# TUMFTM/global_racetrajectory_optimization

Hardware: NVIDIA H100
Metric: min-curv QPs/sec (N=1000 closed track, batched) (higher is better)
Workload: dtype f64

## Files before the change

global_racetrajectory_optimization_b200/batch.py:

```python
from __future__ import annotations

import ctypes
import functools
import math
from typing import Optional, Union

import torch

from . import _lib

_GRID_Y_MAX = 65535
N_MIN = 80
STATUS_TEXT = {
    0: "ok",
    1: "Problem not solvable, track might be too small to run with current safety distance!",
    2: "interior-point iteration cap reached",
    3: "numerical breakdown (non-positive pivot)",
    4: "curvature rows still violated after the curvature-row phase (constraints inconsistent)",
    -1: "unsupported track size",
}

F_SCALE = 2.0
VP_DECEL_SLICE_UPPER = 1

_WS = {}

SLAB_VECTORS = ("H DIAG DFW DBW LFW INVD TII RHOP RHOM PX PY NX NY MX MY XP YP SX SY KREF LB UB F "
                "T0 T1 T2 T3 T4 T5 ALPHA LU LL RD RHS DX DD DLU DLL SU SL ISU ISL HBSRC "
                "S3 S4 L3 L4 KL WK EDX T3K T4K VV IH").split()
HB_PITCH = 34
ZB_PITCH = 108


def mincurv_slab_layout(n_max: int) -> dict:
    np_ = ((n_max + 31) // 32) * 32 + 64
    nb_max = max(1, (n_max - 32 + 31) // 32)
    o = len(SLAB_VECTORS) * np_
    o_zb = o
    o += n_max * ZB_PITCH
    o_hb = o
    o += np_ * HB_PITCH
    o_tiles = o
    o += np_ * 67
    return dict(np=np_, nb_max=nb_max, o_zb=o_zb, o_hb=o_hb, o_tiles=o_tiles, stride=(o + 15) & ~15)


def _require_cuda() -> None:
    if not torch.cuda.is_available():
        raise _lib.MinCurvLibError("global_racetrajectory_optimization_b200 needs a CUDA device (H100, sm_90a); "
                                   "there is no CPU fallback")


def _ptr(t: Optional[torch.Tensor]):
    return ctypes.c_void_p(t.data_ptr()) if t is not None else None


def _stream():
    return ctypes.c_void_p(torch.cuda.current_stream().cuda_stream)


def _device_guard(fn):
    @functools.wraps(fn)
    def wrapper(*args, **kwargs):
        dev = next((a.device for a in list(args) + list(kwargs.values()) if isinstance(a, torch.Tensor) and a.is_cuda), None)
        if dev is None:
            return fn(*args, **kwargs)
# ... 697 lines not shown
```

global_racetrajectory_optimization_b200/csrc/mincurv_ipm.cu:

```cuda
#include <cstdio>
#include <cstdlib>
#include "mincurv_ops.cuh"

namespace mc {

constexpr unsigned FULL = 0xffffffffu;
constexpr int IP_THREADS = 64;
constexpr int SUB = 8;
constexpr int VBP = 12;
constexpr int FROW = 34;
constexpr int HB_SLOTS = 2;
constexpr int HO_SLOTS = 2;
constexpr int LROW = 33;
#ifndef MC_LT_SLOTS
#define MC_LT_SLOTS 3
#endif
constexpr int LT_SLOTS = MC_LT_SLOTS;
constexpr int GT_SLOTS = 6 - LT_SLOTS;
constexpr int RING_UNITS = LT_SLOTS + GT_SLOTS;
constexpr int QDEPTH = 16;
constexpr int LT_UNIT_DOUBLES = SUB * LROW;
constexpr int GT_UNIT_DOUBLES = SUB * FROW;
constexpr unsigned HB_UNIT_BYTES = SUB * HB_PITCH * sizeof(double);

__device__ __forceinline__ void dmma(double (&c)[2], double a, double b) {
    asm volatile("mma.sync.aligned.m8n8k4.row.col.f64.f64.f64.f64 {%0,%1}, {%2}, {%3}, {%0,%1};\n"
                 : "+d"(c[0]), "+d"(c[1]) : "d"(a), "d"(b));
}

__device__ __forceinline__ uint32_t smem_u32(const void *p) { return (uint32_t)__cvta_generic_to_shared(p); }
__device__ __forceinline__ void mbar_init(uint64_t *bar, unsigned count) {
    asm volatile("mbarrier.init.shared::cta.b64 [%0], %1;" ::"r"(smem_u32(bar)), "r"(count) : "memory");
}
__device__ __forceinline__ void mbar_expect_tx(uint64_t *bar, unsigned bytes) {
    asm volatile("mbarrier.arrive.expect_tx.shared::cta.b64 _, [%0], %1;" ::"r"(smem_u32(bar)), "r"(bytes) : "memory");
}
__device__ __forceinline__ void mbar_arrive(uint64_t *bar) {
    asm volatile("mbarrier.arrive.shared::cta.b64 _, [%0];" ::"r"(smem_u32(bar)) : "memory");
}
#ifndef MC_WAIT_MODE
#define MC_WAIT_MODE 1
#endif
#ifndef MC_RELAXED_BACKOFF_NS
#define MC_RELAXED_BACKOFF_NS 250
#endif
// ... 92 lines not shown
            double lt[LT_SLOTS][LT_UNIT_DOUBLES];
            double gt[GT_SLOTS][GT_UNIT_DOUBLES];
            double q[QDEPTH * SUB];
        } sw;
        double win[hband_win_doubles(IP_THREADS)];
    } u;
    union {
        double Ss[32 * 33];
        double sfrag[20 * 32];
    } s;
    double wS[32], gs[32], part[2][32];
    double red[32];
    uint64_t hb_full[HB_SLOTS], ho_full[HO_SLOTS], ho_empty[HO_SLOTS], ring_full[RING_UNITS];
    unsigned ring_phase[2];
    int prog[4];
    int flag;
    int next;
};

struct Factor {
    const double *HB;
    const double *DD;
    double *LT, *GT;
    int n, NA;
};

__device__ __forceinline__ Factor make_factor(double *slab, const Layout &L, int n, const double *HB) {
    Factor F;
    F.HB = HB;
    F.DD = vec(slab, L, V_DD);
    F.LT = slab + L.o_tiles;
    F.GT = F.LT + (size_t)L.np * LROW;
    F.n = n;
    F.NA = n - 32;
    return F;
}

__device__ __forceinline__ int lt_slot(int c, int m) { return LROW * c + ((m + 3 * c - 1) & 31); }
__device__ __forceinline__ double lt_entry(const double *unit, int c, int m) {
    return (c < m && m <= c + 32) ? unit[lt_slot(c, m)] : 0.0;
}

__device__ __forceinline__ int blk(int I, int J) { return (I * (I + 1)) / 2 + J; }

__device__ __noinline__ bool factor_chain(IpShared &sh, const double *__restrict__ HBp, const double *__restrict__ DD, double *__restrict__ LTp, double *__restrict__ GTp, const int NA, const double *__restrict__ g, unsigned tick) {
    const int lane = threadIdx.x & 31;
    const int gq = lane >> 2, q = lane & 3;
    const int nunits = (NA + SUB - 1) / SUB;
    const uint64_t pol = l2_evict_normal_policy();
    double W[10][2];
#pragma unroll
    for (int b = 0; b < 10; ++b) { W[b][0] = 0.0; W[b][1] = 0.0; }
    double gv = (lane < NA) ? g[lane] : 0.0;
    double gcur = (32 + lane < NA) ? g[32 + lane] : 0.0;
    double gnext = (64 + lane < NA) ? g[64 + lane] : 0.0;
    double ddcur = (lane < NA) ? DD[lane] : 0.0;
    double ddnext = (32 + lane < NA) ? DD[32 + lane] : 0.0;
    bool ok = true;
    if (lane == 0) {
        mbar_expect_tx(&sh.hb_full[tick % HB_SLOTS], HB_UNIT_BYTES);
        tma_load_1d(sh.u.f.hb[tick % HB_SLOTS], HBp, HB_UNIT_BYTES, &sh.hb_full[tick % HB_SLOTS], pol);
    }
    SEG_BEGIN();
    for (int t = 0; t < nunits; ++t) {
// ... 111 lines not shown
            }
        }
#pragma unroll
        for (int I = 0; I < 4; ++I)
#pragma unroll
            for (int J = 0; J <= I; ++J) {
                double c[2] = {0.0, 0.0};
                if (I < 3) { c[0] = W[blk(I + 1, J + 1)][0]; c[1] = W[blk(I + 1, J + 1)][1]; }
                dmma(c, af[I][0], bf[J][0]);
                dmma(c, af[I][1], bf[J][1]);
                W[blk(I, J)][0] = c[0]; W[blk(I, J)][1] = c[1];
            }
        {
            const double up = __shfl_sync(FULL, gv, (lane + 8) & 31), en = __shfl_sync(FULL, gv2, (lane - 24) & 31);
            gv = (lane < 24) ? up : en;
        }
        __syncwarp();
        SEG(12);
        if (lane == 0) mbar_arrive(&sh.ho_full[ls]);
    }
    return ok;
}

__device__ __noinline__ void factor_fill(IpShared &sh, const double *__restrict__ HBp, double *__restrict__ LTp, double *__restrict__ GTp, const int NA, const double *__restrict__ g, unsigned tick) {
    const int lane = threadIdx.x & 31;
    const int gq = lane >> 2, q = lane & 3;
    const int nunits = (NA + SUB - 1) / SUB;
    double G[4][4][2];
#pragma unroll
    for (int I = 0; I < 4; ++I)
#pragma unroll
        for (int J = 0; J < 4; ++J) { G[I][J][0] = 0.0; G[I][J][1] = 0.0; }
    double gsacc = 0.0;
    double *gb = sh.u.f.gb;
    for (int t = 0; t < nunits; ++t) {
        const unsigned ht = tick + t, ls = ht % HO_SLOTS;
        const int k0 = t * SUB;
#pragma unroll
        for (int I = 0; I < 4; ++I)
            *reinterpret_cast<double2 *>(&gb[(8 * I + gq) * VBP + 2 * q]) = make_double2(G[I][0][0], G[I][0][1]);
        __syncwarp();
        double gp[8];
#pragma unroll
        for (int j = 0; j < 8; j += 2) {
            const double2 uu = *reinterpret_cast<const double2 *>(&gb[lane * VBP + j]);
            gp[j] = uu.x; gp[j + 1] = uu.y;
        }
// ... 2 lines not shown
#pragma unroll
            for (int j = 0; j < 8; ++j) {
                const int k = k0 + j;
                double yv = 0.0;
                if (k < NA) {
                    if (k <= lane) yv = HBp[(size_t)(NA + lane) * HB_PITCH + (k + 32 - lane)];
                    else if (k >= NA + lane - 32) yv = HBp[(size_t)k * HB_PITCH + (NA + lane - k)];
                }
                gp[j] = yv - gp[j];
            }
        } else {
#pragma unroll
            for (int j = 0; j < 8; ++j) gp[j] = -gp[j];
        }
        __syncwarp();
        PROF_T0(tw2);
        mbar_wait_relaxed(&sh.ho_full[ls], (ht / HO_SLOTS) & 1u);
        PROF_ADD1(20, tw2);
        const Handoff &ho = sh.u.f.ho[ls];
#pragma unroll
        for (int m = 0; m < 7; ++m)
#pragma unroll
            for (int j = m + 1; j < 8; ++j) gp[j] = fma(-gp[m], ho.l11[j * 8 + m], gp[j]);
        double *gtp = GTp + (size_t)k0 * FROW;
#pragma unroll
        for (int j = 0; j < 8; ++j) {
            st_stream(gtp + j * FROW + lane, gp[j]);
            gsacc = fma(gp[j], ho.w[j] * ho.y[j], gsacc);
        }
        if (lane < 8) {
            const double w = ho.w[lane];
            *reinterpret_cast<double2 *>(gtp + lane * FROW + 32) = make_double2(w * ho.y[lane], w);
        }
#pragma unroll
        for (int j = 0; j < 8; j += 2) *reinterpret_cast<double2 *>(&gb[lane * VBP + j]) = make_double2(gp[j], gp[j + 1]);
        __syncwarp();
        PROF_T0(tw3);
        double af[4][2], bf[4][2], wq[2];
#pragma unroll
        for (int ks = 0; ks < 2; ++ks) {
            wq[ks] = ho.w[4 * ks + q];
#pragma unroll
            for (int I = 0; I < 4; ++I) {
                af[I][ks] = gb[(8 * I + gq) * VBP + 4 * ks + q];
                bf[I][ks] = ho.vb[(8 * I + gq) * VBP + 4 * ks + q];
            }
        }
#pragma unroll
        for (int I = 0; I < 4; ++I)
#pragma unroll
            for (int J = 0; J < 4; ++J) {
                double c[2] = {0.0, 0.0};
                if (J < 3) { c[0] = G[I][J + 1][0]; c[1] = G[I][J + 1][1]; }
                dmma(c, af[I][0], bf[J][0]);
                dmma(c, af[I][1], bf[J][1]);
// ... 17 lines not shown
            for (int J = 0; J <= I; ++J)
                *reinterpret_cast<double2 *>(&sh.s.sfrag[(blk(I, J) * 32 + lane) * 2]) = make_double2(c2[J][0], c2[J][1]);
        }
        __syncwarp();
        PROF_ADD1(21, tw3);
        if (lane == 0) mbar_arrive(&sh.ho_empty[ls]);
    }
    sh.gs[lane] = g[NA + lane] - gsacc;
}

__device__ __forceinline__ unsigned factor_units(int n) { return (unsigned)((n - 32 + SUB - 1) / SUB); }
__device__ __noinline__ bool factor(IpShared &sh, double *slab, const Layout &L, int n, const double *HB, const double *g, unsigned tick) {
    const Factor F = make_factor(slab, L, n, HB);
    const int NA = F.NA;
    const int warp = threadIdx.x >> 5, lane = threadIdx.x & 31;
    for (int e = threadIdx.x; e < 20 * 32; e += IP_THREADS) sh.s.sfrag[e] = 0.0;
    fence_proxy_async();
    __syncthreads();
    PROF_T0(tc0);
    if (warp == 0) {
        if (!factor_chain(sh, F.HB, F.DD, F.LT, F.GT, NA, g, tick)) sh.flag = 1;
        PROF_ADD(1, tc0);
    } else {
        factor_fill(sh, F.HB, F.LT, F.GT, NA, g, tick);
        PROF_ADD1(13, tc0);
    }
    PROF_T0(tc1);
    double sf[20];
    if (warp == 1) {
#pragma unroll
        for (int e = 0; e < 20; ++e) sf[e] = sh.s.sfrag[((e >> 1) * 32 + lane) * 2 + (e & 1)];
    }
    double sv[16];
#pragma unroll
    for (int i = 0; i < 16; ++i) {
        const int e = threadIdx.x + i * IP_THREADS;
        const int r = e >> 5, c = e & 31;
        const int lo = min(r, c), dist = abs(r - c);
        sv[i] = F.HB[(size_t)(NA + lo) * HB_PITCH + dist];
        if (r == c) sv[i] += F.DD[NA + r];
    }
    __syncthreads();
#pragma unroll
    for (int i = 0; i < 16; ++i) {
        const int e = threadIdx.x + i * IP_THREADS;
        sh.s.Ss[(e >> 5) * 33 + (e & 31)] = sv[i];
    }
// ... 58 lines not shown
        phase ^= 1u << sl;
        return buf + sl * UNIT_DOUBLES;
    }
    __device__ __forceinline__ void close() { sh.ring_phase[WHO] = phase; }
};
using LtRing = RingT<LT_SLOTS, 0, LT_UNIT_DOUBLES, 0>;
using GtRing = RingT<GT_SLOTS, LT_SLOTS, GT_UNIT_DOUBLES, 1>;

__device__ __forceinline__ void prog_publish(int *p, int v) { asm volatile("st.release.cta.shared.s32 [%0], %1;" ::"r"(smem_u32(p)), "r"(v) : "memory"); }
__device__ __forceinline__ int prog_read(const int *p) {
    int v;
    asm volatile("ld.acquire.cta.shared.s32 %0, [%1];" : "=r"(v) : "r"(smem_u32(p)) : "memory");
    return v;
}
template <bool BACKOFF = false>
__device__ __forceinline__ void prog_wait(IpShared &sh, const int *p, int need) {
    for (int spin = 0; spin < (1 << 18); ++spin) {
        if (prog_read(p) >= need) return;
        if (BACKOFF) __nanosleep(MC_RELAXED_BACKOFF_NS);
    }
    sh.flag = 1;
}

__device__ __noinline__ void sweep_forward(IpShared &sh, const double *__restrict__ HBp, double *__restrict__ LTp, double *__restrict__ GTp, const int NA, const double *__restrict__ g) {
    const int lane = threadIdx.x & 31;
    const int gq = lane >> 2, q = lane & 3;
    const int nunits = (NA + SUB - 1) / SUB;
    constexpr int AHEAD = LT_SLOTS - 1;
    LtRing R(sh, &sh.u.sw.lt[0][0]);
    if (lane == 0)
        for (int u = 0; u < AHEAD && u < nunits; ++u) R.issue(u, u, LTp);
    double acc[4];
#pragma unroll
    for (int I = 0; I < 4; ++I) acc[I] = (8 * I + gq < NA) ? g[8 * I + gq] : 0.0;
    double gcur = (32 + lane < NA) ? g[32 + lane] : 0.0;
    double gnext = (64 + lane < NA) ? g[64 + lane] : 0.0;
    int sl = 0, sn = AHEAD % LT_SLOTS;
    for (int u = 0; u < nunits; ++u, sl = (sl == LT_SLOTS - 1) ? 0 : sl + 1, sn = (sn == LT_SLOTS - 1) ? 0 : sn + 1) {
        const int k0 = u * SUB;
        if (u > 0 && (u & 3) == 0) {
            gcur = gnext;
            const int idx = k0 + 64 + lane;
            gnext = (idx < NA) ? g[idx] : 0.0;
        }
        if ((u & 7) == 0 && u >= 8) prog_wait(sh, &sh.prog[1], u - 8);
        const double *lt = R.wait(sl);
        const double ge = __shfl_sync(FULL, gcur, ((u & 3) << 3) + gq);
// ... 3 lines not shown
            a[I][0] = lt_entry(lt, q, 8 * I + gq);
            a[I][1] = lt_entry(lt, 4 + q, 8 * I + gq);
        }
        const double wl = lt[gq * LROW + 32];
        const double b0 = __shfl_sync(FULL, acc[0], 4 * q), b1 = __shfl_sync(FULL, acc[0], 16 + 4 * q);
        double y0[2] = {acc[0], acc[0]}, y1[2] = {0.0, 0.0};
        dmma(y0, a[0][0], b0);
        dmma(y1, a[0][1], b1);
        const double y = y0[0] + y1[0];
        const double n0 = -__shfl_sync(FULL, y, 4 * q), n1 = -__shfl_sync(FULL, y, 16 + 4 * q);
        double nw[4];
#pragma unroll
        for (int I = 0; I < 4; ++I) {
            const double c = (I < 3) ? acc[I + 1] : ge;
            double c0[2] = {c, c}, c1[2] = {0.0, 0.0};
            dmma(c0, a[I + 1][0], n0);
            dmma(c1, a[I + 1][1], n1);
            nw[I] = c0[0] + c1[0];
        }
        if (q == 0) {
            const bool in = (k0 + gq < NA);
            const double z = in ? y * wl : 0.0;
            sh.u.sw.q[(u & (QDEPTH - 1)) * SUB + gq] = z;
            if (in) GTp[(size_t)(k0 + gq) * FROW + 32] = z;
        }
#pragma unroll
        for (int I = 0; I < 4; ++I) acc[I] = nw[I];
        __syncwarp();
        if (lane == 0) {
            prog_publish(&sh.prog[0], u + 1);
            if (u + AHEAD < nunits) R.issue(u + AHEAD, sn, LTp);
        }
    }
    R.close();
    fence_proxy_async();
}

__device__ __noinline__ void sweep_sep_rhs(IpShared &sh, const double *__restrict__ HBp, double *__restrict__ LTp, double *__restrict__ GTp, const int NA, const double *__restrict__ g) {
    const int lane = threadIdx.x & 31;
    const int nunits = (NA + SUB - 1) / SUB;
    constexpr int AHEAD = GT_SLOTS - 1;
    GtRing R(sh, &sh.u.sw.gt[0][0]);
    if (lane == 0)
        for (int u = 0; u < AHEAD && u < nunits; ++u) R.issue(u, u, GTp);
    double s0 = 0.0, s1 = 0.0;
    const double gsl = g[NA + lane];
    int sl = 0, sn = AHEAD % GT_SLOTS;
    for (int u = 0; u < nunits; ++u, sl = (sl == GT_SLOTS - 1) ? 0 : sl + 1, sn = (sn == GT_SLOTS - 1) ? 0 : sn + 1) {
        const double *gt = R.wait(sl) + lane;
        prog_wait<true>(sh, &sh.prog[0], u + 1);
        const double *zq = &sh.u.sw.q[(u & (QDEPTH - 1)) * SUB];
#pragma unroll
        for (int s2 = 0; s2 < SUB; s2 += 2) {
            s0 = fma(gt[s2 * FROW], zq[s2], s0);
            s1 = fma(gt[(s2 + 1) * FROW], zq[s2 + 1], s1);
        }
        __syncwarp();
        if (lane == 0) {
            prog_publish(&sh.prog[1], u + 1);
            if (u + AHEAD < nunits) R.issue(u + AHEAD, sn, GTp);
        }
    }
    R.close();
    sh.gs[lane] = gsl - (s0 + s1);
}

__device__ __noinline__ void sweep_sep_solve(IpShared &sh, const double *__restrict__ HBp, double *__restrict__ LTp, double *__restrict__ GTp, const int NA, double *__restrict__ x) {
    const int lane = threadIdx.x & 31;
    const int nunits = (NA + SUB - 1) / SUB;
    constexpr int AHEAD = GT_SLOTS - 1;
    GtRing R(sh, &sh.u.sw.gt[0][0]);
    const int U0 = nunits - 1;
    if (lane == 0)
        for (int i = 0; i < AHEAD && i < nunits; ++i) R.issue(U0 - i, i, GTp);
    double a = sh.gs[lane];
#pragma unroll 4
    for (int k = 0; k < 32; ++k) {
        const double yk = __shfl_sync(FULL, a, k);
        const double l = (lane > k) ? sh.s.Ss[lane * 33 + k] : 0.0;
        a = fma(-l, yk, a);
    }
    a *= sh.wS[lane];
#pragma unroll 4
    for (int k = 31; k >= 0; --k) {
        const double xk = __shfl_sync(FULL, a, k);
        const double l = (lane < k) ? sh.s.Ss[k * 33 + lane] : 0.0;
        a = fma(-l, xk, a);
    }
    x[NA + lane] = a;
    const int kl = lane & 7, qr = lane >> 3;
    double xq[8];
#pragma unroll
    for (int i = 0; i < 8; ++i) xq[i] = __shfl_sync(FULL, a, 8 * qr + i);
    int sl = 0, sn = AHEAD % GT_SLOTS;
    for (int i = 0; i < nunits; ++i, sl = (sl == GT_SLOTS - 1) ? 0 : sl + 1, sn = (sn == GT_SLOTS - 1) ? 0 : sn + 1) {
        const int k = (U0 - i) * SUB + kl;
        if ((i & 7) == 0 && i >= 8) prog_wait<true>(sh, &sh.prog[2], i - 8);
        const double *gt = R.wait(sl) + kl * FROW;
        const double2 zw = *reinterpret_cast<const double2 *>(&gt[32]);
        double c0 = 0.0, c1 = 0.0;
#pragma unroll
        for (int e = 0; e < 8; e += 2) {
            const double2 gg = *reinterpret_cast<const double2 *>(&gt[8 * qr + e]);
            c0 = fma(gg.x, xq[e], c0);
            c1 = fma(gg.y, xq[e + 1], c1);
        }
        double c = c0 + c1;
        c += __shfl_xor_sync(FULL, c, 8);
        c += __shfl_xor_sync(FULL, c, 16);
        if (qr == 0) sh.u.sw.q[(i & (QDEPTH - 1)) * SUB + kl] = (k < NA) ? fma(-c, zw.y, zw.x) : 0.0;
        __syncwarp();
        if (lane == 0) {
            prog_publish(&sh.prog[3], i + 1);
            if (i + AHEAD < nunits) R.issue(U0 - i - AHEAD, sn, GTp);
        }
    }
    R.close();
}

__device__ __noinline__ void sweep_backward(IpShared &sh, const double *__restrict__ HBp, double *__restrict__ LTp, double *__restrict__ GTp, const int NA, double *__restrict__ x) {
    const int lane = threadIdx.x & 31;
    const int gq = lane >> 2, q = lane & 3;
    const int nunits = (NA + SUB - 1) / SUB;
    constexpr int AHEAD = LT_SLOTS - 1;
    LtRing R(sh, &sh.u.sw.lt[0][0]);
    const int U0 = nunits - 1;
    if (lane == 0)
        for (int i = 0; i < AHEAD && i < nunits; ++i) R.issue(U0 - i, i, LTp);
    double nbx[8];
#pragma unroll
    for (int i = 0; i < 8; ++i) nbx[i] = 0.0;
    int sl = 0, sn = AHEAD % LT_SLOTS;
    for (int i = 0; i < nunits; ++i, sl = (sl == LT_SLOTS - 1) ? 0 : sl + 1, sn = (sn == LT_SLOTS - 1) ? 0 : sn + 1) {
        const int k0 = (U0 - i) * SUB;
        const double *lt = R.wait(sl);
        double a[10];
#pragma unroll
        for (int c = 0; c < 10; ++c) a[c] = lt_entry(lt, gq, 4 * c + q);
        double c0[2] = {0.0, 0.0}, c1[2] = {0.0, 0.0};
#pragma unroll
        for (int e = 2; e < 8; e += 2) {
            dmma(c0, a[2 + e], nbx[e]);
            dmma(c1, a[3 + e], nbx[e + 1]);
        }
        dmma(c0, a[2], nbx[0]);
        dmma(c1, a[3], nbx[1]);
        prog_wait(sh, &sh.prog[3], i + 1);
        const double t1 = sh.u.sw.q[(i & (QDEPTH - 1)) * SUB + gq];
        const double uu = t1 + (c0[0] + c1[0]);
        const double u0 = __shfl_sync(FULL, uu, 4 * q), u1 = __shfl_sync(FULL, uu, 16 + 4 * q);
        double d0[2] = {uu, uu}, d1[2] = {0.0, 0.0};
        dmma(d0, a[0], u0);
        dmma(d1, a[1], u1);
        const double x1 = d0[0] + d1[0];
        if (q == 0 && k0 + gq < NA) x[k0 + gq] = x1;
#pragma unroll
        for (int e = 7; e >= 2; --e) nbx[e] = nbx[e - 2];
        nbx[0] = -__shfl_sync(FULL, x1, 4 * q);
        nbx[1] = -__shfl_sync(FULL, x1, 16 + 4 * q);
        __syncwarp();
        if (lane == 0) {
            prog_publish(&sh.prog[2], i + 1);
            if (i + AHEAD < nunits) R.issue(U0 - i - AHEAD, sn, LTp);
        }
    }
    R.close();
}

__device__ __noinline__ void solve(IpShared &sh, double *slab, const Layout &L, int n, const double *g, double *x, bool fused) {
    const Factor F = make_factor(slab, L, n, nullptr);
    const int warp = threadIdx.x >> 5;
    if (threadIdx.x < 4) sh.prog[threadIdx.x] = 0;
    fence_proxy_async();
    __syncthreads();
    if (!fused) {
        PROF_T0(t0);
        if (warp == 0) sweep_forward(sh, F.HB, F.LT, F.GT, F.NA, g);
        else sweep_sep_rhs(sh, F.HB, F.LT, F.GT, F.NA, g);
        __syncthreads();
        PROF_ADD1(2, t0);
    }
    PROF_T0(t3);
    if (warp == 1) sweep_sep_solve(sh, F.HB, F.LT, F.GT, F.NA, x);
    else sweep_backward(sh, F.HB, F.LT, F.GT, F.NA, x);
    __syncthreads();
    PROF_ADD1(8, t3);
}

__device__ void band_matvec(const double *__restrict__ HB, const double *__restrict__ v, double *__restrict__ out, int n) {
    for (int i = threadIdx.x; i < n; i += IP_THREADS) {
        const double *row = HB + (size_t)i * HB_PITCH;
        double s = row[0] * v[i];
        int j = i;
        for (int k = 1; k <= HBW; ++k) {
            j = (j + 1 == n) ? 0 : j + 1;
            s = fma(row[k], v[j], s);
        }
        j = i;
        for (int k = 1; k <= HBW; ++k) {
            j = (j == 0) ? n - 1 : j - 1;
            s = fma(HB[(size_t)j * HB_PITCH + k], v[j], s);
        }
        out[i] = s;
    }
}

__device__ __forceinline__ void ip_init_shared(IpShared &sh) {
    if (threadIdx.x == 0) {
        for (int i = 0; i < HB_SLOTS; ++i) mbar_init(&sh.hb_full[i], 1);
        for (int i = 0; i < HO_SLOTS; ++i) { mbar_init(&sh.ho_full[i], 1); mbar_init(&sh.ho_empty[i], 1); }
        for (int i = 0; i < RING_UNITS; ++i) mbar_init(&sh.ring_full[i], 1);
        sh.ring_phase[0] = 0; sh.ring_phase[1] = 0;
        asm volatile("fence.mbarrier_init.release.cluster;" ::: "memory");
    }
    __syncthreads();
}

__global__ void __launch_bounds__(IP_THREADS, 8)
mincurv_pdip_kernel(int B, int n_max, const int32_t *__restrict__ n_pts, double *__restrict__ ws, Layout L,
                    PdipParams prm, double *__restrict__ alpha_out, int32_t *__restrict__ status,
                    int32_t *__restrict__ iters_out, int *__restrict__ work_counter) {
    extern __shared__ __align__(16) unsigned char smem_raw[];
    IpShared &sh = *reinterpret_cast<IpShared *>(smem_raw);
#ifdef MC_DEBUG_SM_LIMIT
    {
        unsigned smid;
        asm volatile("mov.u32 %0, %%smid;" : "=r"(smid));
        if (smid >= MC_DEBUG_SM_LIMIT) return;
    }
#endif
    ip_init_shared(sh);
    unsigned tick = 0;

    for (;;) {
        __syncthreads();
        if (threadIdx.x == 0) sh.next = atomicAdd(work_counter, 1);
        __syncthreads();
        const int b = sh.next;
        if (b >= B) break;
        const int n = n_pts ? n_pts[b] : n_max;
        double *aout = alpha_out + (size_t)b * n_max;
        if (status[b] != 0) {
            for (int i = threadIdx.x; i < n_max; i += IP_THREADS) aout[i] = 0.0;
            if (iters_out && threadIdx.x == 0) iters_out[b] = 0;
            continue;
        }
        PROF_T0(tq0);
        double *slab = ws + (size_t)b * L.stride;
        const double *HB = ws + (size_t)*band_owner(slab, L) * L.stride + L.o_hb;
        const double *__restrict__ LB = vec(slab, L, V_LB), *__restrict__ UB = vec(slab, L, V_UB), *__restrict__ F = vec(slab, L, V_F);
        double *__restrict__ AL = vec(slab, L, V_ALPHA), *__restrict__ LU = vec(slab, L, V_LU), *__restrict__ LL = vec(slab, L, V_LL), *__restrict__ RD = vec(slab, L, V_RD);
        double *__restrict__ RHS = vec(slab, L, V_RHS), *__restrict__ DX = vec(slab, L, V_DX), *__restrict__ DD = vec(slab, L, V_DD);
        double *__restrict__ TU = vec(slab, L, V_DLU), *__restrict__ TL = vec(slab, L, V_DLL), *__restrict__ SU = vec(slab, L, V_SU), *__restrict__ SL = vec(slab, L, V_SL);
        double *__restrict__ ISU = vec(slab, L, V_ISU), *__restrict__ ISL = vec(slab, L, V_ISL);
        double *G0 = vec(slab, L, V_T0);
        if (threadIdx.x == 0) sh.flag = 0;

        for (int i = threadIdx.x; i < n; i += IP_THREADS) AL[i] = 0.5 * (LB[i] + UB[i]);
        __syncthreads();
        band_matvec(HB, AL, G0, n);
        __syncthreads();
        double gmax = 0.0, fmaxv = 0.0;
#pragma unroll 1
        for (int i = threadIdx.x; i < n; i += IP_THREADS) {
            const double gi = G0[i] + F[i];
            G0[i] = gi;
            gmax = fmax(gmax, fabs(gi));
            fmaxv = fmax(fmaxv, fabs(F[i]));
        }
        gmax = block_reduce<1>(gmax, sh.red);
        fmaxv = block_reduce<1>(fmaxv, sh.red);
        const double lam0 = prm.lam0_rel * gmax + 1e-300;
        double musum = 0.0;
#pragma unroll 1
        for (int i = threadIdx.x; i < n; i += IP_THREADS) {
            const double gi = G0[i];
            const double lu = fmax(-gi, 0.0) + lam0, ll = fmax(gi, 0.0) + lam0;
            const double rd = gi + lu - ll;
            LU[i] = lu; LL[i] = ll;
            RD[i] = rd;
            const double a = AL[i];
            const double su = UB[i] - a, sl = a - LB[i];
            const double isu = 1.0 / su, isl = 1.0 / sl;
            SU[i] = su; SL[i] = sl;
            ISU[i] = isu; ISL[i] = isl;
            DD[i] = lu * isu + ll * isl; RHS[i] = -rd + lu - ll;
            musum += su * lu + sl * ll;
        }
        musum = block_reduce<0>(musum, sh.red);
        const double mu0 = musum / (2.0 * n);
        const double rd_tol = prm.rd_rel * (fmaxv + gmax) + 1e-300;
        double mu = mu0;
        int it = 0;
        int result = 2;

        constexpr int VG = 4, VS = VG * IP_THREADS;
        for (it = 0; it < prm.max_iter; ++it) {
            PROF_T0(tf0);
            const bool fok = factor(sh, slab, L, n, HB, RHS, tick);
            tick += factor_units(n);
            if (!fok) { result = 3; break; }
            PROF_ADD(10, tf0);
            PROF_T0(ts0);
            solve(sh, slab, L, n, RHS, DX, true);
            PROF_ADD(6, ts0);
            PROF_T0(tv2);
            double rp = 0.0, rdl = 0.0, c00 = 0.0, c01 = 0.0, c10 = 0.0, c11 = 0.0;
#pragma unroll 1
            for (int i0 = threadIdx.x; i0 < n; i0 += VS) {
                double su[VG], sl[VG], lu[VG], ll[VG], dx[VG], isu[VG], isl[VG];
#pragma unroll
                for (int k = 0; k < VG; ++k) {
                    const int i = min(i0 + k * IP_THREADS, n - 1);
                    su[k] = SU[i]; sl[k] = SL[i]; lu[k] = LU[i]; ll[k] = LL[i]; dx[k] = DX[i]; isu[k] = ISU[i]; isl[k] = ISL[i];
                }
#pragma unroll
                for (int k = 0; k < VG; ++k) {
                    if (i0 + k * IP_THREADS < n) {
                        const double p = dx[k] * isu[k], m = dx[k] * isl[k];
                        rp = fmax(rp, fmax(p, -m));
                        rdl = fmax(rdl, fmax(1.0 - p, 1.0 + m));
                        const double dlu = lu[k] * (p - 1.0), dll = -ll[k] * (1.0 + m);
                        c00 += su[k] * lu[k] + sl[k] * ll[k];
                        c01 += su[k] * dlu + sl[k] * dll;
                        c10 += dx[k] * (ll[k] - lu[k]);
                        c11 += dx[k] * (dll - dlu);
                    }
                }
            }
            rp = block_reduce<1>(rp, sh.red);
            rdl = block_reduce<1>(rdl, sh.red);
            double ap = (rp > 1.0) ? 1.0 / rp : 1.0, ad = (rdl > 1.0) ? 1.0 / rdl : 1.0;
            c00 = block_reduce<0>(c00, sh.red); c01 = block_reduce<0>(c01, sh.red);
            c10 = block_reduce<0>(c10, sh.red); c11 = block_reduce<0>(c11, sh.red);
            const double mua = (c00 + ad * c01 + ap * c10 + ap * ad * c11) / (2.0 * n);
            double sigma = mua / mu;
            sigma = sigma * sigma * sigma;
            const double smu = sigma * mu;
            PROF_ADD(17, tv2);
            PROF_T0(tv3);
#pragma unroll 1
            for (int i0 = threadIdx.x; i0 < n; i0 += VS) {
                double su[VG], sl[VG], lu[VG], ll[VG], dx[VG], isu[VG], isl[VG], rd[VG];
#pragma unroll
                for (int k = 0; k < VG; ++k) {
                    const int i = min(i0 + k * IP_THREADS, n - 1);
                    su[k] = SU[i]; sl[k] = SL[i]; lu[k] = LU[i]; ll[k] = LL[i]; dx[k] = DX[i]; isu[k] = ISU[i]; isl[k] = ISL[i]; rd[k] = RD[i];
                }
#pragma unroll
                for (int k = 0; k < VG; ++k) {
                    const int i = i0 + k * IP_THREADS;
                    if (i < n) {
                        const double dlu = lu[k] * (dx[k] * isu[k] - 1.0), dll = -ll[k] * (1.0 + dx[k] * isl[k]);
                        const double tu = smu - su[k] * lu[k] + dx[k] * dlu;
                        const double tl = smu - sl[k] * ll[k] - dx[k] * dll;
                        TU[i] = tu; TL[i] = tl;
                        RHS[i] = -rd[k] - tu * isu[k] + tl * isl[k];
                    }
                }
            }
            __syncthreads();
            PROF_ADD(18, tv3);
            PROF_T0(ts1);
            solve(sh, slab, L, n, RHS, DX, false);
            PROF_ADD(7, ts1);
            PROF_T0(tv4);
            rp = 0.0; rdl = 0.0;
#pragma unroll 1
            for (int i0 = threadIdx.x; i0 < n; i0 += VS) {
                double lu[VG], ll[VG], dx[VG], isu[VG], isl[VG], tu[VG], tl[VG];
#pragma unroll
                for (int k = 0; k < VG; ++k) {
                    const int i = min(i0 + k * IP_THREADS, n - 1);
                    lu[k] = LU[i]; ll[k] = LL[i]; dx[k] = DX[i]; isu[k] = ISU[i]; isl[k] = ISL[i]; tu[k] = TU[i]; tl[k] = TL[i];
                }
#pragma unroll
                for (int k = 0; k < VG; ++k) {
                    if (i0 + k * IP_THREADS < n) {
                        const double dlu = (tu[k] + lu[k] * dx[k]) * isu[k], dll = (tl[k] - ll[k] * dx[k]) * isl[k];
                        rp = fmax(rp, fmax(dx[k] * isu[k], -dx[k] * isl[k]));
                        rdl = fmax(rdl, fmax(-dlu / lu[k], -dll / ll[k]));
                    }
                }
            }
            rp = block_reduce<1>(rp, sh.red);
            rdl = block_reduce<1>(rdl, sh.red);
            ap = (prm.eta < rp) ? prm.eta / rp : 1.0;
            ad = (prm.eta < rdl) ? prm.eta / rdl : 1.0;
            PROF_ADD(15, tv4);
            PROF_T0(tv5);
            double musum2 = 0.0, rdmax = 0.0, dxmax = 0.0, amax = 0.0;
            constexpr int VG2 = 2, VS2 = VG2 * IP_THREADS;
#pragma unroll 1
            for (int i0 = threadIdx.x; i0 < n; i0 += VS2) {
                double su[VG2], sl[VG2], lu[VG2], ll[VG2], dx[VG2], isu[VG2], isl[VG2], tu[VG2], tl[VG2], al[VG2], rd[VG2], rh[VG2], dd[VG2];
#pragma unroll
                for (int k = 0; k < VG2; ++k) {
                    const int i = min(i0 + k * IP_THREADS, n - 1);
                    su[k] = SU[i]; sl[k] = SL[i]; lu[k] = LU[i]; ll[k] = LL[i]; dx[k] = DX[i]; isu[k] = ISU[i]; isl[k] = ISL[i];
                    tu[k] = TU[i]; tl[k] = TL[i]; al[k] = AL[i]; rd[k] = RD[i]; rh[k] = RHS[i]; dd[k] = DD[i];
                }
#pragma unroll
                for (int k = 0; k < VG2; ++k) {
                    const int i = i0 + k * IP_THREADS;
                    if (i < n) {
                        const double dlu = (tu[k] + lu[k] * dx[k]) * isu[k], dll = (tl[k] - ll[k] * dx[k]) * isl[k];
                        const double an = al[k] + ap * dx[k], lun = lu[k] + ad * dlu, lln = ll[k] + ad * dll;
                        const double sun = su[k] - ap * dx[k], sln = sl[k] + ap * dx[k];
                        const double rdn = rd[k] + ap * (rh[k] - dd[k] * dx[k]) + ad * (dlu - dll);
                        const double isun = 1.0 / sun, isln = 1.0 / sln;
                        AL[i] = an; LU[i] = lun; LL[i] = lln; RD[i] = rdn; SU[i] = sun; SL[i] = sln;
                        ISU[i] = isun; ISL[i] = isln;
                        DD[i] = lun * isun + lln * isln; RHS[i] = -rdn + lun - lln;
                        musum2 += sun * lun + sln * lln;
                        rdmax = fmax(rdmax, fabs(rdn));
                        dxmax = fmax(dxmax, fabs(dx[k]));
                        amax = fmax(amax, fabs(an));
                    }
                }
            }
            mu = block_reduce<0>(musum2, sh.red) / (2.0 * n);
            rdmax = block_reduce<1>(rdmax, sh.red);
            PROF_ADD(0, tv5);
            bool settled = true;
            if (prm.dx_rel > 0.0 && mu <= prm.mu_rel * mu0) {
                dxmax = block_reduce<1>(dxmax, sh.red);
                amax = block_reduce<1>(amax, sh.red);
                settled = ap * dxmax <= prm.dx_rel * fmax(amax, 0.01);
            }
            if (mu <= prm.mu_rel * mu0 && rdmax <= rd_tol && settled) { result = 0; ++it; break; }
            if (mu <= 1e-4 * prm.mu_rel * mu0) { result = (rdmax <= 1e3 * rd_tol) ? 0 : 2; ++it; break; }
        }
        __syncthreads();
        for (int i = threadIdx.x; i < n_max; i += IP_THREADS) aout[i] = (i < n) ? AL[i] : 0.0;
        if (threadIdx.x == 0) {
            status[b] = result;
// ... 276 lines not shown
```

global_racetrajectory_optimization_b200/csrc/mincurv_ws.cuh:

```cuda
#pragma once
#include "common.cuh"

namespace mc {

enum Vec : int {
    V_H = 0, V_DIAG, V_DFW, V_DBW, V_LFW, V_INVD, V_TII, V_RHOP, V_RHOM,
    V_PX, V_PY, V_NX, V_NY, V_MX, V_MY, V_XP, V_YP, V_SX, V_SY, V_KREF,
    V_LB, V_UB, V_F,
    V_T0, V_T1, V_T2, V_T3, V_T4, V_T5,
    V_ALPHA, V_LU, V_LL, V_RD, V_RHS, V_DX, V_DD, V_DLU, V_DLL, V_SU, V_SL,
    V_ISU, V_ISL, V_HBSRC,
    V_S3, V_S4, V_L3, V_L4, V_KL, V_WK, V_EDX, V_T3K, V_T4K, V_VV,
    V_IH,
    NUM_VEC
};

struct Layout {
    int n_max;
    int np;
    int nb_max;
    size_t o_zb, o_hb, o_tiles, stride;
};

__host__ __device__ inline Layout make_layout(int n_max) {
    Layout L;
    L.n_max = n_max;
    L.np = ((n_max + 31) / 32) * 32 + 64;
    L.nb_max = (n_max - 32 + 31) / 32;
    if (L.nb_max < 1) L.nb_max = 1;
    size_t o = (size_t)NUM_VEC * L.np;
    L.o_zb = o;
    o += (size_t)n_max * ZB_PITCH;
    L.o_hb = o;
    o += (size_t)L.np * HB_PITCH;
    L.o_tiles = o;
    o += (size_t)L.np * 67;
    L.stride = (o + 15) & ~(size_t)15;
    return L;
}

struct PdipParams {
    int max_iter;
    double mu_rel;
    double rd_rel;
    double eta;
    double dx_rel;
    double lam0_rel;
};

__device__ __forceinline__ double *vec(double *slab, const Layout &L, int v) { return slab + (size_t)v * L.np; }

__device__ __forceinline__ int32_t *band_owner(double *slab, const Layout &L) { return reinterpret_cast<int32_t *>(vec(slab, L, V_HBSRC)); }

}
```

Baseline: 54190.

## Shrink GT tile rows, move z/w out of tiles, recompute IPM scratch on the fly

GT tile rows shrink from 34 to 32 doubles using a rotated slot index that avoids bank conflicts. The z vector now goes to its own Z vector, and the w scaling is applied in the backward sweep, which reads w from the LT tile. The IPM vector loops stop storing ISU/ISL/TU/TL and recompute reciprocals and centring terms from SU/SL. The affine direction is kept in a separate DXA vector so the corrector can rebuild its terms. The aim is to cut global memory traffic in the banded solve and the per-iteration elementwise passes, at the cost of extra divisions and changed rounding.

```diff
diff --git a/global_racetrajectory_optimization_b200/batch.py b/global_racetrajectory_optimization_b200/batch.py
--- a/global_racetrajectory_optimization_b200/batch.py
+++ b/global_racetrajectory_optimization_b200/batch.py
@@ -27,7 +27,7 @@
 
 SLAB_VECTORS = ("H DIAG DFW DBW LFW INVD TII RHOP RHOM PX PY NX NY MX MY XP YP SX SY KREF LB UB F "
                 "T0 T1 T2 T3 T4 T5 ALPHA LU LL RD RHS DX DD DLU DLL SU SL ISU ISL HBSRC "
-                "S3 S4 L3 L4 KL WK EDX T3K T4K VV IH").split()
+                "S3 S4 L3 L4 KL WK EDX T3K T4K VV IH DXA Z").split()
 HB_PITCH = 34
 ZB_PITCH = 108
 
@@ -41,7 +41,7 @@
     o_hb = o
     o += np_ * HB_PITCH
     o_tiles = o
-    o += np_ * 67
+    o += np_ * 65
     return dict(np=np_, nb_max=nb_max, o_zb=o_zb, o_hb=o_hb, o_tiles=o_tiles, stride=(o + 15) & ~15)
 
 
diff --git a/global_racetrajectory_optimization_b200/csrc/mincurv_ipm.cu b/global_racetrajectory_optimization_b200/csrc/mincurv_ipm.cu
--- a/global_racetrajectory_optimization_b200/csrc/mincurv_ipm.cu
+++ b/global_racetrajectory_optimization_b200/csrc/mincurv_ipm.cu
@@ -8,7 +8,7 @@
 constexpr int IP_THREADS = 64;
 constexpr int SUB = 8;
 constexpr int VBP = 12;
-constexpr int FROW = 34;
+constexpr int GROW = 32;
 constexpr int HB_SLOTS = 2;
 constexpr int HO_SLOTS = 2;
 constexpr int LROW = 33;
@@ -20,7 +20,7 @@
 constexpr int RING_UNITS = LT_SLOTS + GT_SLOTS;
 constexpr int QDEPTH = 16;
 constexpr int LT_UNIT_DOUBLES = SUB * LROW;
-constexpr int GT_UNIT_DOUBLES = SUB * FROW;
+constexpr int GT_UNIT_DOUBLES = SUB * GROW;
 constexpr unsigned HB_UNIT_BYTES = SUB * HB_PITCH * sizeof(double);
 
 __device__ __forceinline__ void dmma(double (&c)[2], double a, double b) {
@@ -159,6 +159,7 @@
     const double *HB;
     const double *DD;
     double *LT, *GT;
+    double *Z;
     int n, NA;
 };
 
@@ -168,6 +169,7 @@
     F.DD = vec(slab, L, V_DD);
     F.LT = slab + L.o_tiles;
     F.GT = F.LT + (size_t)L.np * LROW;
+    F.Z = vec(slab, L, V_Z);
     F.n = n;
     F.NA = n - 32;
     return F;
@@ -177,6 +179,7 @@
 __device__ __forceinline__ double lt_entry(const double *unit, int c, int m) {
     return (c < m && m <= c + 32) ? unit[lt_slot(c, m)] : 0.0;
 }
+__device__ __forceinline__ int gt_slot(int c, int r) { return GROW * c + ((r + 2 * c) & 31); }
 
 __device__ __forceinline__ int blk(int I, int J) { return (I * (I + 1)) / 2 + J; }
 
@@ -334,7 +337,7 @@
     return ok;
 }
 
-__device__ __noinline__ void factor_fill(IpShared &sh, const double *__restrict__ HBp, double *__restrict__ LTp, double *__restrict__ GTp, const int NA, const double *__restrict__ g, unsigned tick) {
+__device__ __noinline__ void factor_fill(IpShared &sh, const double *__restrict__ HBp, double *__restrict__ GTp, double *__restrict__ Z, const int NA, const double *__restrict__ g, unsigned tick) {
     const int lane = threadIdx.x & 31;
     const int gq = lane >> 2, q = lane & 3;
     const int nunits = (NA + SUB - 1) / SUB;
@@ -383,15 +386,15 @@
         for (int m = 0; m < 7; ++m)
 #pragma unroll
             for (int j = m + 1; j < 8; ++j) gp[j] = fma(-gp[m], ho.l11[j * 8 + m], gp[j]);
-        double *gtp = GTp + (size_t)k0 * FROW;
+        double *gtp = GTp + (size_t)k0 * GROW;
 #pragma unroll
         for (int j = 0; j < 8; ++j) {
-            st_stream(gtp + j * FROW + lane, gp[j]);
+            st_stream(gtp + gt_slot(j, lane), gp[j]);
             gsacc = fma(gp[j], ho.w[j] * ho.y[j], gsacc);
         }
-        if (lane < 8) {
+        if (lane < 8 && k0 + lane < NA) {
             const double w = ho.w[lane];
-            *reinterpret_cast<double2 *>(gtp + lane * FROW + 32) = make_double2(w * ho.y[lane], w);
+            Z[k0 + lane] = w * ho.y[lane];
         }
 #pragma unroll
         for (int j = 0; j < 8; j += 2) *reinterpret_cast<double2 *>(&gb[lane * VBP + j]) = make_double2(gp[j], gp[j + 1]);
@@ -455,7 +458,7 @@
         if (!factor_chain(sh, F.HB, F.DD, F.LT, F.GT, NA, g, tick)) sh.flag = 1;
         PROF_ADD(1, tc0);
     } else {
-        factor_fill(sh, F.HB, F.LT, F.GT, NA, g, tick);
+        factor_fill(sh, F.HB, F.GT, F.Z, NA, g, tick);
         PROF_ADD1(13, tc0);
     }
     PROF_T0(tc1);
@@ -560,7 +563,7 @@
     sh.flag = 1;
 }
 
-__device__ __noinline__ void sweep_forward(IpShared &sh, const double *__restrict__ HBp, double *__restrict__ LTp, double *__restrict__ GTp, const int NA, const double *__restrict__ g) {
+__device__ __noinline__ void sweep_forward(IpShared &sh, double *__restrict__ LTp, double *__restrict__ Z, const int NA, const double *__restrict__ g) {
     const int lane = threadIdx.x & 31;
     const int gq = lane >> 2, q = lane & 3;
     const int nunits = (NA + SUB - 1) / SUB;
@@ -610,7 +613,7 @@
             const bool in = (k0 + gq < NA);
             const double z = in ? y * wl : 0.0;
             sh.u.sw.q[(u & (QDEPTH - 1)) * SUB + gq] = z;
-            if (in) GTp[(size_t)(k0 + gq) * FROW + 32] = z;
+            if (in) Z[k0 + gq] = z;
         }
 #pragma unroll
         for (int I = 0; I < 4; ++I) acc[I] = nw[I];
@@ -621,10 +624,9 @@
         }
     }
     R.close();
-    fence_proxy_async();
-}
-
-__device__ __noinline__ void sweep_sep_rhs(IpShared &sh, const double *__restrict__ HBp, double *__restrict__ LTp, double *__restrict__ GTp, const int NA, const double *__restrict__ g) {
+}
+
+__device__ __noinline__ void sweep_sep_rhs(IpShared &sh, double *__restrict__ GTp, const int NA, const double *__restrict__ g) {
     const int lane = threadIdx.x & 31;
     const int nunits = (NA + SUB - 1) / SUB;
     constexpr int AHEAD = GT_SLOTS - 1;
@@ -635,13 +637,13 @@
     const double gsl = g[NA + lane];
     int sl = 0, sn = AHEAD % GT_SLOTS;
     for (int u = 0; u < nunits; ++u, sl = (sl == GT_SLOTS - 1) ? 0 : sl + 1, sn = (sn == GT_SLOTS - 1) ? 0 : sn + 1) {
-        const double *gt = R.wait(sl) + lane;
+        const double *gt = R.wait(sl);
         prog_wait<true>(sh, &sh.prog[0], u + 1);
         const double *zq = &sh.u.sw.q[(u & (QDEPTH - 1)) * SUB];
 #pragma unroll
         for (int s2 = 0; s2 < SUB; s2 += 2) {
-            s0 = fma(gt[s2 * FROW], zq[s2], s0);
-            s1 = fma(gt[(s2 + 1) * FROW], zq[s2 + 1], s1);
+            s0 = fma(gt[gt_slot(s2, lane)], zq[s2], s0);
+            s1 = fma(gt[gt_slot(s2 + 1, lane)], zq[s2 + 1], s1);
         }
         __syncwarp();
         if (lane == 0) {
@@ -653,7 +655,7 @@
     sh.gs[lane] = gsl - (s0 + s1);
 }
 
-__device__ __noinline__ void sweep_sep_solve(IpShared &sh, const double *__restrict__ HBp, double *__restrict__ LTp, double *__restrict__ GTp, const int NA, double *__restrict__ x) {
+__device__ __noinline__ void sweep_sep_solve(IpShared &sh, double *__restrict__ GTp, const int NA, double *__restrict__ x) {
     const int lane = threadIdx.x & 31;
     const int nunits = (NA + SUB - 1) / SUB;
     constexpr int AHEAD = GT_SLOTS - 1;
@@ -676,7 +678,7 @@
         a = fma(-l, xk, a);
     }
     x[NA + lane] = a;
-    const int kl = lane & 7, qr = lane >> 3;
+    const int kl = lane & 7, qr = lane >> 3, rot = 8 * qr + 2 * kl;
     double xq[8];
 #pragma unroll
     for (int i = 0; i < 8; ++i) xq[i] = __shfl_sync(FULL, a, 8 * qr + i);
@@ -684,19 +686,18 @@
     for (int i = 0; i < nunits; ++i, sl = (sl == GT_SLOTS - 1) ? 0 : sl + 1, sn = (sn == GT_SLOTS - 1) ? 0 : sn + 1) {
         const int k = (U0 - i) * SUB + kl;
         if ((i & 7) == 0 && i >= 8) prog_wait<true>(sh, &sh.prog[2], i - 8);
-        const double *gt = R.wait(sl) + kl * FROW;
-        const double2 zw = *reinterpret_cast<const double2 *>(&gt[32]);
+        const double *gt = R.wait(sl) + kl * GROW;
         double c0 = 0.0, c1 = 0.0;
 #pragma unroll
         for (int e = 0; e < 8; e += 2) {
-            const double2 gg = *reinterpret_cast<const double2 *>(&gt[8 * qr + e]);
+            const double2 gg = *reinterpret_cast<const double2 *>(&gt[(rot + e) & 31]);
             c0 = fma(gg.x, xq[e], c0);
             c1 = fma(gg.y, xq[e + 1], c1);
         }
         double c = c0 + c1;
         c += __shfl_xor_sync(FULL, c, 8);
         c += __shfl_xor_sync(FULL, c, 16);
-        if (qr == 0) sh.u.sw.q[(i & (QDEPTH - 1)) * SUB + kl] = (k < NA) ? fma(-c, zw.y, zw.x) : 0.0;
+        if (qr == 0) sh.u.sw.q[(i & (QDEPTH - 1)) * SUB + kl] = (k < NA) ? c : 0.0;
         __syncwarp();
         if (lane == 0) {
             prog_publish(&sh.prog[3], i + 1);
@@ -706,7 +707,7 @@
     R.close();
 }
 
-__device__ __noinline__ void sweep_backward(IpShared &sh, const double *__restrict__ HBp, double *__restrict__ LTp, double *__restrict__ GTp, const int NA, double *__restrict__ x) {
+__device__ __noinline__ void sweep_backward(IpShared &sh, double *__restrict__ LTp, const double *__restrict__ Z, const int NA, double *__restrict__ x) {
     const int lane = threadIdx.x & 31;
     const int gq = lane >> 2, q = lane & 3;
     const int nunits = (NA + SUB - 1) / SUB;
@@ -718,10 +719,20 @@
     double nbx[8];
 #pragma unroll
     for (int i = 0; i < 8; ++i) nbx[i] = 0.0;
+    const int zb = 32 * (U0 >> 2) + lane;
+    double zcur = (zb < NA) ? Z[zb] : 0.0;
+    double znext = (zb >= 32) ? Z[zb - 32] : 0.0;
     int sl = 0, sn = AHEAD % LT_SLOTS;
     for (int i = 0; i < nunits; ++i, sl = (sl == LT_SLOTS - 1) ? 0 : sl + 1, sn = (sn == LT_SLOTS - 1) ? 0 : sn + 1) {
-        const int k0 = (U0 - i) * SUB;
+        const int u = U0 - i, k0 = u * SUB;
+        if (i > 0 && (u & 3) == 3) {
+            zcur = znext;
+            const int idx = 32 * (u >> 2) - 32 + lane;
+            znext = (idx >= 0) ? Z[idx] : 0.0;
+        }
+        const double zl = __shfl_sync(FULL, zcur, ((u & 3) << 3) + gq);
         const double *lt = R.wait(sl);
+        const double wl = lt[gq * LROW + 32];
         double a[10];
 #pragma unroll
         for (int c = 0; c < 10; ++c) a[c] = lt_entry(lt, gq, 4 * c + q);
@@ -734,7 +745,7 @@
         dmma(c0, a[2], nbx[0]);
         dmma(c1, a[3], nbx[1]);
         prog_wait(sh, &sh.prog[3], i + 1);
-        const double t1 = sh.u.sw.q[(i & (QDEPTH - 1)) * SUB + gq];
+        const double t1 = fma(-sh.u.sw.q[(i & (QDEPTH - 1)) * SUB + gq], wl, zl);
         const double uu = t1 + (c0[0] + c1[0]);
         const double u0 = __shfl_sync(FULL, uu, 4 * q), u1 = __shfl_sync(FULL, uu, 16 + 4 * q);
         double d0[2] = {uu, uu}, d1[2] = {0.0, 0.0};
@@ -763,14 +774,14 @@
     __syncthreads();
     if (!fused) {
         PROF_T0(t0);
-        if (warp == 0) sweep_forward(sh, F.HB, F.LT, F.GT, F.NA, g);
-        else sweep_sep_rhs(sh, F.HB, F.LT, F.GT, F.NA, g);
+        if (warp == 0) sweep_forward(sh, F.LT, F.Z, F.NA, g);
+        else sweep_sep_rhs(sh, F.GT, F.NA, g);
         __syncthreads();
         PROF_ADD1(2, t0);
     }
     PROF_T0(t3);
-    if (warp == 1) sweep_sep_solve(sh, F.HB, F.LT, F.GT, F.NA, x);
-    else sweep_backward(sh, F.HB, F.LT, F.GT, F.NA, x);
+    if (warp == 1) sweep_sep_solve(sh, F.GT, F.NA, x);
+    else sweep_backward(sh, F.LT, F.Z, F.NA, x);
     __syncthreads();
     PROF_ADD1(8, t3);
 }
@@ -802,6 +813,24 @@
         asm volatile("fence.mbarrier_init.release.cluster;" ::: "memory");
     }
     __syncthreads();
+}
+
+__device__ __forceinline__ double barrier_diag(double lu, double ll, double isu, double isl) {
+    return __fma_rn(lu, isu, __dmul_rn(ll, isl));
+}
+__device__ __forceinline__ void centring(double su, double sl, double lu, double ll, double dxa, double isu, double isl,
+                                         double smu, double &tu, double &tl) {
+    const double dlu = __dmul_rn(lu, __fma_rn(dxa, isu, -1.0)), dll = -__dmul_rn(ll, __fma_rn(dxa, isl, 1.0));
+    tu = __fma_rn(dxa, dlu, __fma_rn(-su, lu, smu));
+    tl = __fma_rn(-dxa, dll, __fma_rn(-sl, ll, smu));
+}
+__device__ __forceinline__ double corrector_rhs(double rd, double tu, double tl, double isu, double isl) {
+    return __fma_rn(tl, isl, __fma_rn(-tu, isu, -rd));
+}
+__device__ __forceinline__ void corrector_steps(double lu, double ll, double dx, double tu, double tl, double isu, double isl,
+                                                double &dlu, double &dll) {
+    dlu = __dmul_rn(__fma_rn(lu, dx, tu), isu);
+    dll = __dmul_rn(__fma_rn(-ll, dx, tl), isl);
 }
 
 __global__ void __launch_bounds__(IP_THREADS, 8)
@@ -838,9 +867,8 @@
         const double *HB = ws + (size_t)*band_owner(slab, L) * L.stride + L.o_hb;
         const double *__restrict__ LB = vec(slab, L, V_LB), *__restrict__ UB = vec(slab, L, V_UB), *__restrict__ F = vec(slab, L, V_F);
         double *__restrict__ AL = vec(slab, L, V_ALPHA), *__restrict__ LU = vec(slab, L, V_LU), *__restrict__ LL = vec(slab, L, V_LL), *__restrict__ RD = vec(slab, L, V_RD);
-        double *__restrict__ RHS = vec(slab, L, V_RHS), *__restrict__ DX = vec(slab, L, V_DX), *__restrict__ DD = vec(slab, L, V_DD);
-        double *__restrict__ TU = vec(slab, L, V_DLU), *__restrict__ TL = vec(slab, L, V_DLL), *__restrict__ SU = vec(slab, L, V_SU), *__restrict__ SL = vec(slab, L, V_SL);
-        double *__restrict__ ISU = vec(slab, L, V_ISU), *__restrict__ ISL = vec(slab, L, V_ISL);
+        double *__restrict__ RHS = vec(slab, L, V_RHS), *__restrict__ DX = vec(slab, L, V_DX), *__restrict__ DXA = vec(slab, L, V_DXA);
+        double *__restrict__ DD = vec(slab, L, V_DD), *__restrict__ SU = vec(slab, L, V_SU), *__restrict__ SL = vec(slab, L, V_SL);
         double *G0 = vec(slab, L, V_T0);
         if (threadIdx.x == 0) sh.flag = 0;
 
@@ -871,8 +899,7 @@
             const double su = UB[i] - a, sl = a - LB[i];
             const double isu = 1.0 / su, isl = 1.0 / sl;
             SU[i] = su; SL[i] = sl;
-            ISU[i] = isu; ISL[i] = isl;
-            DD[i] = lu * isu + ll * isl; RHS[i] = -rd + lu - ll;
+            DD[i] = barrier_diag(lu, ll, isu, isl); RHS[i] = -rd + lu - ll;
             musum += su * lu + sl * ll;
         }
         musum = block_reduce<0>(musum, sh.red);
@@ -890,22 +917,23 @@
             if (!fok) { result = 3; break; }
             PROF_ADD(10, tf0);
             PROF_T0(ts0);
-            solve(sh, slab, L, n, RHS, DX, true);
+            solve(sh, slab, L, n, RHS, DXA, true);
             PROF_ADD(6, ts0);
             PROF_T0(tv2);
             double rp = 0.0, rdl = 0.0, c00 = 0.0, c01 = 0.0, c10 = 0.0, c11 = 0.0;
 #pragma unroll 1
             for (int i0 = threadIdx.x; i0 < n; i0 += VS) {
-                double su[VG], sl[VG], lu[VG], ll[VG], dx[VG], isu[VG], isl[VG];
+                double su[VG], sl[VG], lu[VG], ll[VG], dx[VG];
 #pragma unroll
                 for (int k = 0; k < VG; ++k) {
                     const int i = min(i0 + k * IP_THREADS, n - 1);
-                    su[k] = SU[i]; sl[k] = SL[i]; lu[k] = LU[i]; ll[k] = LL[i]; dx[k] = DX[i]; isu[k] = ISU[i]; isl[k] = ISL[i];
+                    su[k] = SU[i]; sl[k] = SL[i]; lu[k] = LU[i]; ll[k] = LL[i]; dx[k] = DXA[i];
                 }
 #pragma unroll
                 for (int k = 0; k < VG; ++k) {
                     if (i0 + k * IP_THREADS < n) {
-                        const double p = dx[k] * isu[k], m = dx[k] * isl[k];
+                        const double isu = 1.0 / su[k], isl = 1.0 / sl[k];
+                        const double p = dx[k] * isu, m = dx[k] * isl;
                         rp = fmax(rp, fmax(p, -m));
                         rdl = fmax(rdl, fmax(1.0 - p, 1.0 + m));
                         const double dlu = lu[k] * (p - 1.0), dll = -ll[k] * (1.0 + m);
@@ -929,21 +957,20 @@
             PROF_T0(tv3);
 #pragma unroll 1
             for (int i0 = threadIdx.x; i0 < n; i0 += VS) {
-                double su[VG], sl[VG], lu[VG], ll[VG], dx[VG], isu[VG], isl[VG], rd[VG];
+                double su[VG], sl[VG], lu[VG], ll[VG], dxa[VG], rd[VG];
 #pragma unroll
                 for (int k = 0; k < VG; ++k) {
                     const int i = min(i0 + k * IP_THREADS, n - 1);
-                    su[k] = SU[i]; sl[k] = SL[i]; lu[k] = LU[i]; ll[k] = LL[i]; dx[k] = DX[i]; isu[k] = ISU[i]; isl[k] = ISL[i]; rd[k] = RD[i];
+                    su[k] = SU[i]; sl[k] = SL[i]; lu[k] = LU[i]; ll[k] = LL[i]; dxa[k] = DXA[i]; rd[k] = RD[i];
                 }
 #pragma unroll
                 for (int k = 0; k < VG; ++k) {
                     const int i = i0 + k * IP_THREADS;
                     if (i < n) {
-                        const double dlu = lu[k] * (dx[k] * isu[k] - 1.0), dll = -ll[k] * (1.0 + dx[k] * isl[k]);
-                        const double tu = smu - su[k] * lu[k] + dx[k] * dlu;
-                        const double tl = smu - sl[k] * ll[k] - dx[k] * dll;
-                        TU[i] = tu; TL[i] = tl;
-                        RHS[i] = -rd[k] - tu * isu[k] + tl * isl[k];
+                        const double isu = 1.0 / su[k], isl = 1.0 / sl[k];
+                        double tu, tl;
+                        centring(su[k], sl[k], lu[k], ll[k], dxa[k], isu, isl, smu, tu, tl);
+                        RHS[i] = corrector_rhs(rd[k], tu, tl, isu, isl);
                     }
                 }
             }
@@ -956,17 +983,20 @@
             rp = 0.0; rdl = 0.0;
 #pragma unroll 1
             for (int i0 = threadIdx.x; i0 < n; i0 += VS) {
-                double lu[VG], ll[VG], dx[VG], isu[VG], isl[VG], tu[VG], tl[VG];
+                double su[VG], sl[VG], lu[VG], ll[VG], dx[VG], dxa[VG];
 #pragma unroll
                 for (int k = 0; k < VG; ++k) {
                     const int i = min(i0 + k * IP_THREADS, n - 1);
-                    lu[k] = LU[i]; ll[k] = LL[i]; dx[k] = DX[i]; isu[k] = ISU[i]; isl[k] = ISL[i]; tu[k] = TU[i]; tl[k] = TL[i];
+                    su[k] = SU[i]; sl[k] = SL[i]; lu[k] = LU[i]; ll[k] = LL[i]; dx[k] = DX[i]; dxa[k] = DXA[i];
                 }
 #pragma unroll
                 for (int k = 0; k < VG; ++k) {
                     if (i0 + k * IP_THREADS < n) {
-                        const double dlu = (tu[k] + lu[k] * dx[k]) * isu[k], dll = (tl[k] - ll[k] * dx[k]) * isl[k];
-                        rp = fmax(rp, fmax(dx[k] * isu[k], -dx[k] * isl[k]));
+                        const double isu = 1.0 / su[k], isl = 1.0 / sl[k];
+                        double tu, tl, dlu, dll;
+                        centring(su[k], sl[k], lu[k], ll[k], dxa[k], isu, isl, smu, tu, tl);
+                        corrector_steps(lu[k], ll[k], dx[k], tu, tl, isu, isl, dlu, dll);
+                        rp = fmax(rp, fmax(dx[k] * isu, -dx[k] * isl));
                         rdl = fmax(rdl, fmax(-dlu / lu[k], -dll / ll[k]));
                     }
                 }
@@ -981,25 +1011,27 @@
             constexpr int VG2 = 2, VS2 = VG2 * IP_THREADS;
 #pragma unroll 1
             for (int i0 = threadIdx.x; i0 < n; i0 += VS2) {
-                double su[VG2], sl[VG2], lu[VG2], ll[VG2], dx[VG2], isu[VG2], isl[VG2], tu[VG2], tl[VG2], al[VG2], rd[VG2], rh[VG2], dd[VG2];
+                double su[VG2], sl[VG2], lu[VG2], ll[VG2], dx[VG2], dxa[VG2], al[VG2], rd[VG2];
 #pragma unroll
                 for (int k = 0; k < VG2; ++k) {
                     const int i = min(i0 + k * IP_THREADS, n - 1);
-                    su[k] = SU[i]; sl[k] = SL[i]; lu[k] = LU[i]; ll[k] = LL[i]; dx[k] = DX[i]; isu[k] = ISU[i]; isl[k] = ISL[i];
-                    tu[k] = TU[i]; tl[k] = TL[i]; al[k] = AL[i]; rd[k] = RD[i]; rh[k] = RHS[i]; dd[k] = DD[i];
+                    su[k] = SU[i]; sl[k] = SL[i]; lu[k] = LU[i]; ll[k] = LL[i]; dx[k] = DX[i]; dxa[k] = DXA[i];
+                    al[k] = AL[i]; rd[k] = RD[i];
                 }
 #pragma unroll
                 for (int k = 0; k < VG2; ++k) {
                     const int i = i0 + k * IP_THREADS;
                     if (i < n) {
-                        const double dlu = (tu[k] + lu[k] * dx[k]) * isu[k], dll = (tl[k] - ll[k] * dx[k]) * isl[k];
+                        const double isu = 1.0 / su[k], isl = 1.0 / sl[k];
+                        double tu, tl, dlu, dll;
+                        centring(su[k], sl[k], lu[k], ll[k], dxa[k], isu, isl, smu, tu, tl);
+                        const double dd = barrier_diag(lu[k], ll[k], isu, isl), rh = corrector_rhs(rd[k], tu, tl, isu, isl);
+                        corrector_steps(lu[k], ll[k], dx[k], tu, tl, isu, isl, dlu, dll);
                         const double an = al[k] + ap * dx[k], lun = lu[k] + ad * dlu, lln = ll[k] + ad * dll;
                         const double sun = su[k] - ap * dx[k], sln = sl[k] + ap * dx[k];
-                        const double rdn = rd[k] + ap * (rh[k] - dd[k] * dx[k]) + ad * (dlu - dll);
-                        const double isun = 1.0 / sun, isln = 1.0 / sln;
+                        const double rdn = rd[k] + ap * (rh - dd * dx[k]) + ad * (dlu - dll);
                         AL[i] = an; LU[i] = lun; LL[i] = lln; RD[i] = rdn; SU[i] = sun; SL[i] = sln;
-                        ISU[i] = isun; ISL[i] = isln;
-                        DD[i] = lun * isun + lln * isln; RHS[i] = -rdn + lun - lln;
+                        DD[i] = barrier_diag(lun, lln, 1.0 / sun, 1.0 / sln); RHS[i] = -rdn + lun - lln;
                         musum2 += sun * lun + sln * lln;
                         rdmax = fmax(rdmax, fabs(rdn));
                         dxmax = fmax(dxmax, fabs(dx[k]));
diff --git a/global_racetrajectory_optimization_b200/csrc/mincurv_ws.cuh b/global_racetrajectory_optimization_b200/csrc/mincurv_ws.cuh
--- a/global_racetrajectory_optimization_b200/csrc/mincurv_ws.cuh
+++ b/global_racetrajectory_optimization_b200/csrc/mincurv_ws.cuh
@@ -12,6 +12,7 @@
     V_ISU, V_ISL, V_HBSRC,
     V_S3, V_S4, V_L3, V_L4, V_KL, V_WK, V_EDX, V_T3K, V_T4K, V_VV,
     V_IH,
+    V_DXA, V_Z,
     NUM_VEC
 };
 
@@ -34,7 +35,7 @@
     L.o_hb = o;
     o += (size_t)L.np * HB_PITCH;
     L.o_tiles = o;
-    o += (size_t)L.np * 67;
+    o += (size_t)L.np * 65;
     L.stride = (o + 15) & ~(size_t)15;
     return L;
 }
```

Result: no change. 55060, median of 6 (+1.6%).
